# IvanBanny/para-ortho-pca-bo

Hardware: AMD Instinct MI355X
Metric: BO iterations/sec (incl. GP refit + EI opt), BBOB f15 d=40 (higher is better)
Workload: dtype f64; 1 GPU; configs[1]: PCA_BO on BBOB f15 d=40, budget=450, n_DoE=120, EI, var_threshold=0.95; one run per GPU (run list f15/d40/instances 0..N-1 partitioned by pcabo.sharding), timed steps spread evenly over the 330 BO iterations of the run; num_restarts=10, raw_samples=512, batch_limit=5, maxiter=200, parallelism=run-parallel x1

## Files before the change

para-ortho-pca-bo_amd/csrc/kernels_acq.hip:

```cpp
#include "pcabo_internal.h"
#include "acq_math.h"
#include <algorithm>
#include <cstdlib>
#include <mutex>

#define PSTRIDE PCABO_PSTRIDE

#ifdef PCABO_ACQ_TIMING
__device__ unsigned long long g_acq_stamps[16];
#define STAMP(i) do { if (blockIdx.x == gridDim.x / 2 && blockIdx.y == 0 && threadIdx.x == 0) g_acq_stamps[i] = wall_clock64(); } while (0)
#define STAMP_FIN(i) do { if (blockIdx.y == 0 && threadIdx.x == 0) g_acq_stamps[i] = wall_clock64(); } while (0)
extern "C" int pcabo_debug_acq_stamps(unsigned long long* out16) {
  return hipMemcpyFromSymbol(out16, HIP_SYMBOL(g_acq_stamps), sizeof(g_acq_stamps)) == hipSuccess ? 0 : -3;
}
#else
#define STAMP(i)
#define STAMP_FIN(i)
#endif

__device__ inline void st_wt(double* p, double v) {
  __hip_atomic_store(p, v, __ATOMIC_RELAXED, __HIP_MEMORY_SCOPE_AGENT);
}

template <int SLAB>
__device__ inline int slab_row(int s, int m, int NP) {
  return m < SLAB / 2 ? (SLAB / 2) * s + m : NP - (SLAB / 2) * (s + 1) + (m - SLAB / 2);
}

__device__ void acq_finish_query(const double* base, int S, int k, int q, const double* bounds4, const double* ystats,
                                 const AcqParams& p, double* val, double* grad, double* host_val, double* host_grad,
                                 int lane);

__device__ inline void grad_partial_sum(const double* base, int S, int c, int first, double* gs_out, double* gm_out) {
  double gs = 0.0, gm = 0.0;
  int sl = first;
  for (; sl + 21 < S; sl += 24) {
    double a[8], b[8];
#pragma unroll
    for (int t = 0; t < 8; ++t) {
      a[t] = base[(size_t)(sl + 3 * t) * PSTRIDE + 2 + c];
      b[t] = base[(size_t)(sl + 3 * t) * PSTRIDE + 2 + PCABO_MAXD + c];
    }
#pragma unroll
    for (int t = 0; t < 8; ++t) { gs += a[t]; gm += b[t]; }
  }
  {
    double a[8], b[8];
#pragma unroll
    for (int t = 0; t < 8; ++t) {
      const int si = sl + 3 * t;
      const int sc = si < S ? si : 0;
      a[t] = base[(size_t)sc * PSTRIDE + 2 + c];
      b[t] = base[(size_t)sc * PSTRIDE + 2 + PCABO_MAXD + c];
    }
#pragma unroll
    for (int t = 0; t < 8; ++t) { if (sl + 3 * t < S) { gs += a[t]; gm += b[t]; } }
  }
  *gs_out = gs;
  *gm_out = gm;
}

__device__ void acq_finish_scalar(const double* base, int S, int q, const double* ystats, const AcqParams& p, double* val,
                                  double* host_val, double* coef, int lane);
__device__ void acq_scalar_core(double vv, double mus, int q, double ym, double ysd, const AcqParams& p, double* val,
                                double* host_val, double* coef, int l);
template <int SLAB>
__device__ inline void acq_tail(int combine, double* s_v, double* partial, unsigned int* counters, int q, int S, int k,
                                const double* bounds4, const double* ystats, const AcqParams& prm, double* val,
                                double* grad, double* host_val, double* host_grad, HostMirror* hm,
                                unsigned long long seq, int tid, int w, int l) {
  if (!combine) return;
  int* s_flag = reinterpret_cast<int*>(s_v + SLAB);
  STAMP(6);
  asm volatile("s_waitcnt vmcnt(0)" ::: "memory");
  __syncthreads();
  STAMP(7);
  if (tid == 0) {
    unsigned int t = __hip_atomic_fetch_add(&counters[q], 1u, __ATOMIC_RELAXED, __HIP_MEMORY_SCOPE_AGENT);
    int last = ((t % (unsigned int)S) == (unsigned int)(S - 1));
    if (last) {
      __builtin_amdgcn_fence(__ATOMIC_ACQUIRE, "agent");
      asm volatile("s_waitcnt vmcnt(0)" ::: "memory");
    }
    *s_flag = last;
  }
  __syncthreads();
  if (!*s_flag) return;
  STAMP_FIN(8);
  const double* base = partial + (size_t)q * S * PSTRIDE;
  double* s_fin = s_v + SLAB + 2;
  double* s_coef = s_fin + 6 * PCABO_MAXD;
  double rng_c = 1.0;
  if (w == 0) {
    if (prm.want_grad && l < k) rng_c = bounds4[PCABO_MAXD + l] - bounds4[l];
    acq_finish_scalar(base, S, q, ystats, prm, val, host_val, s_coef, l);
  } else if (prm.want_grad) {
    for (int c = l; c < k; c += 64) {
      double gs, gm;
      grad_partial_sum(base, S, c, w - 1, &gs, &gm);
      s_fin[(w - 1) * 2 * PCABO_MAXD + c] = gs;
      s_fin[(w - 1) * 2 * PCABO_MAXD + PCABO_MAXD + c] = gm;
    }
  }
  __syncthreads();
  STAMP_FIN(13);
  if (w == 0) {
    if (prm.want_grad) {
      const double c_mu = s_coef[0], c_sg = s_coef[1];
      for (int c = l; c < k; c += 64) {
        const double gs = (s_fin[c] + s_fin[2 * PCABO_MAXD + c]) + s_fin[4 * PCABO_MAXD + c];
        const double gm = (s_fin[PCABO_MAXD + c] + s_fin[3 * PCABO_MAXD + c]) + s_fin[5 * PCABO_MAXD + c];
        const double g = __fma_rn(c_mu, gm, c_sg * gs) / (c == l ? rng_c : bounds4[PCABO_MAXD + c] - bounds4[c]);
        grad[(size_t)q * k + c] = g;
        if (host_grad) host_grad[(size_t)q * k + c] = g;
      }
    }
    if (hm && l == 0)
      __hip_atomic_store(const_cast<unsigned long long*>(&hm->qflag[q]), seq, __ATOMIC_RELEASE, __HIP_MEMORY_SCOPE_SYSTEM);
    STAMP_FIN(9);
#ifdef PCABO_ACQ_TIMING
    asm volatile("s_waitcnt vmcnt(0)" ::: "memory");
    STAMP_FIN(10);
#endif
  }
}

#define ACQ_BATCH_PROLOGUE()                                                                                     \
  unsigned run_ = blockIdx.z;                                                                                    \
  int qsel_ = -1;                                                                                                \
  if (ab.table) {                                                                                                \
    const unsigned e_ = reinterpret_cast<const unsigned*>(qa.x)[blockIdx.y];                                     \
    run_ = e_ >> 16; qsel_ = (int)(e_ & 0xffffu);                                                                \
  }                                                                                                              \
  if (ab.zs) {                                                                                                   \
    ZnT = zrun(ZnT, ab.zs, run_); R = zrun(R, ab.zs, run_); alpha = zrun(alpha, ab.zs, run_);                    \
    bounds4 = zrun(bounds4, ab.zs, run_); ystats = zrun(ystats, ab.zs, run_); partial = zrun(partial, ab.zs, run_); \
    counters = zrun(counters, ab.zs, run_); val = zrun(val, ab.zs, run_); grad = zrun(grad, ab.zs, run_);        \
    Xq = zrun(Xq, ab.xq_host ? ab.hzs : ab.zs, run_);                                                            \
    host_val = zrun(host_val, ab.hzs, run_); host_grad = zrun(host_grad, ab.hzs, run_); hm = zrun(hm, ab.hzs, run_); \
    if (ab.k_dev) k = *zrun(ab.k_dev, ab.zs, run_);                                                              \
    if (ab.bestf) prm.best_f = *zrun(ab.bestf, ab.zs, run_);                                                     \
    if (ab.hyp) prm.inv_ls = zrun(ab.hyp, ab.zs, run_)[PCABO_HYP_INV_LS];                                        \
  }                                                                                                              \
  (void)qsel_;

template <int SLAB>
__global__ __launch_bounds__(256) void k_acq_fused(
    QueryArgs qa, const double* __restrict__ Xq, int q_total, int n, int k, int NP, int ld,
    const double* __restrict__ ZnT, const double* __restrict__ R, const double* __restrict__ alpha,
    const double* __restrict__ bounds4, const double* __restrict__ ystats, AcqParams prm, double* partial,
    unsigned int* counters, double* __restrict__ val, double* __restrict__ grad,
    double* host_val, double* host_grad, HostMirror* hm, unsigned long long seq, int combine, int ,
    MailPair* , MailPair* , AcqBatch ab) {
  ACQ_BATCH_PROLOGUE()
  const double inv_ls = prm.inv_ls;
  const int kernel = prm.kernel, want_grad = prm.want_grad;
  extern __shared__ __attribute__((aligned(16))) double s_dyn[];
  double* s_ks = s_dyn;
  double* s_cf = s_dyn + NP;
  double* s_tm = s_dyn + 2 * NP;
  double* s_xn = s_dyn + 3 * NP;
  double* s_v = s_xn + PCABO_MAXD;
  const int tid = threadIdx.x, w = tid >> 6, l = tid & 63;
  const int s = blockIdx.x, q = ab.table ? qsel_ : (int)blockIdx.y, S = gridDim.x;
  double* out = partial + ((size_t)q * S + s) * PSTRIDE;
  STAMP(0);

  if (tid < k) {
    double lo = bounds4[tid], hi = bounds4[PCABO_MAXD + tid];
    double xv = Xq ? Xq[(size_t)q * k + tid] : qa.x[q * k + tid];
    s_xn[tid] = (xv - lo) / (hi - lo);
  }
  __syncthreads();
  STAMP(1);
  for (int j = tid; j < NP; j += 256) {
    double ks = 0.0, cf = 0.0;
    if (j < n) {
      double sq = 0.0;
      for (int c = 0; c < k; ++c) { double dlt = s_xn[c] - ZnT[(size_t)c * ld + j]; sq += dlt * dlt; }
      sq *= inv_ls * inv_ls;
      acq_cov(sq, kernel, &ks, &cf);
      cf = cf * inv_ls * inv_ls;
    }
    s_ks[j] = ks;
    s_cf[j] = cf;
  }
  __syncthreads();
  STAMP(2);
  {
    constexpr int RW = SLAB / 4;
    int ri[RW];
    const double* Rr[RW];
    double acc[RW];
    int imax = 0;
#pragma unroll
    for (int u = 0; u < RW; ++u) {
      ri[u] = slab_row<SLAB>(s, w + 4 * u, NP); Rr[u] = R + (size_t)ri[u] * ld; acc[u] = 0.0; imax = max(imax, ri[u]);
    }
    for (int j = l; j <= imax; j += 64) {
      const double kj = s_ks[j];
#pragma unroll
      for (int u = 0; u < RW; ++u) acc[u] += Rr[u][j] * kj;
    }
#pragma unroll
    for (int u = 0; u < RW; ++u) acc[u] = wave_sum(acc[u]);
    if (l == 0) {
#pragma unroll
      for (int u = 0; u < RW; ++u) s_v[w + 4 * u] = acc[u];
    }
  }
  __syncthreads();
  STAMP(3);
  if (w == 0) {
    double vv = 0.0, mu = 0.0;
    if (l < SLAB) {
      const int i = slab_row<SLAB>(s, l, NP);
      const double vi = s_v[l];
      vv = vi * vi;
      if (i < n) mu = alpha[i] * s_ks[i];
    }
    vv = wave_sum(vv);
    mu = wave_sum(mu);
    if (l == 0) { st_wt(out + 0, vv); st_wt(out + 1, mu); }
  }
  if (want_grad) {
  __syncthreads();
  STAMP(4);
  for (int j = tid; j < NP; j += 256) {
    double wj = 0.0;
#pragma unroll
    for (int m = 0; m < SLAB; ++m) wj += R[(size_t)slab_row<SLAB>(s, m, NP) * ld + j] * s_v[m];
    const bool mine = ((j / (SLAB / 2)) == s) || (((NP - 1 - j) / (SLAB / 2)) == s);
    const double cf = s_cf[j];
    s_tm[j] = (mine && j < n) ? alpha[j] * cf : 0.0;
    s_ks[j] = wj * cf;
  }
  __syncthreads();
  STAMP(5);
  for (int c0 = 0; c0 < k; c0 += 32) {
    double gs[8], gm[8], xc[8];
    const double* zrow[8];
#pragma unroll
    for (int u = 0; u < 8; ++u) {
      const int c = c0 + w + 4 * u;
      const int cc = c < k ? c : 0;
      gs[u] = 0.0; gm[u] = 0.0; xc[u] = s_xn[cc]; zrow[u] = ZnT + (size_t)cc * ld;
    }
    for (int j = l; j < n; j += 64) {
      const double ts = s_ks[j], tm = s_tm[j];
#pragma unroll
      for (int u = 0; u < 8; ++u) {
        const double dlt = xc[u] - zrow[u][j];
        gs[u] += ts * dlt;
        gm[u] += tm * dlt;
      }
    }
#pragma unroll
    for (int u = 0; u < 8; ++u) { gs[u] = wave_sum(gs[u]); gm[u] = wave_sum(gm[u]); }
    if (l == 0) {
#pragma unroll
      for (int u = 0; u < 8; ++u) {
        const int c = c0 + w + 4 * u;
        if (c < k) { st_wt(out + 2 + c, gs[u]); st_wt(out + 2 + PCABO_MAXD + c, gm[u]); }
      }
    }
  }
  }

  acq_tail<SLAB>(combine, s_v, partial, counters, q, S, k, bounds4, ystats, prm, val, grad, host_val, host_grad, hm, seq, tid, w, l);
}

#define FIN_STAGE_PER_WAVE (11 * 2 * 40)
__device__ inline bool acq_server_finisher(const MailPair* rec, int S, int k, int q, unsigned long long seq,
                                           const double* ystats, const AcqParams& prm, double* val, double* grad,
                                           double* host_val, double* host_grad, HostMirror* hm, double rng_c,
                                           double* s_fin, double* s_coef, double* s_stage, int* s_srv,
                                           unsigned long long t0, int w, int l) {
  if (w == 0) {
    const double ym = ystats[0], ysd = ystats[1];
    const void* ptr[8];
    pcabo_u4 o[8];
    const MailPair* mine = rec + (size_t)(l < S ? l : 0) * PSTRIDE;
#pragma unroll
    for (int t = 0; t < 8; ++t) ptr[t] = mine + (t & 1);
    for (;;) {
      ld_pairs_sys8(ptr, o);
      const bool ok = pair_tag(o[0]) == seq && pair_tag(o[1]) == seq;
      if (__all(ok)) break;
      if (__any(wall_clock64() - t0 > PCABO_SERVER_TIMEOUT_TICKS)) { if (l == 0) *s_srv = 1; break; }
      __builtin_amdgcn_s_sleep(1);
    }
    double vm[2] = {l < S ? pair_value(o[0]) : 0.0, l < S ? pair_value(o[1]) : 0.0};
    wave_sum_multi<2>(vm, l);
    constexpr int lane_vv = wave_multi_lane(2, 0), lane_mus = wave_multi_lane(2, 1);
    const double vv = read_lane(vm[0], lane_vv), mus = read_lane(vm[0], lane_mus);
    acq_scalar_core(vv, mus, q, ym, ysd, prm, val, host_val, s_coef, l);
  } else if (prm.want_grad) {
    const int first = w - 1;
    const int ns = first < S ? (S - first + 2) / 3 : 0;
    const int total = ns * 2 * k;
    double* stage = s_stage + (size_t)(w - 1) * FIN_STAGE_PER_WAVE;
    for (int i0 = 0; i0 < total; i0 += 512) {
      const void* ptr[8];
      int item[8];
#pragma unroll
      for (int t = 0; t < 8; ++t) {
        const int i = i0 + l + 64 * t;
        item[t] = i < total ? i : -1;
        const int ii = i < total ? i : 0;
        const int st = ii / (2 * k), rem = ii - st * 2 * k, which = rem >= k, c = rem - which * k;
        ptr[t] = rec + (size_t)(first + 3 * st) * PSTRIDE + 2 + which * PCABO_MAXD + c;
      }
      pcabo_u4 o[8];
      for (;;) {
        ld_pairs_sys8(ptr, o);
        bool ok = true;
#pragma unroll
        for (int t = 0; t < 8; ++t) ok = ok && (item[t] < 0 || pair_tag(o[t]) == seq);
        if (__all(ok)) break;
        if (__any(wall_clock64() - t0 > PCABO_SERVER_TIMEOUT_TICKS)) { if (l == 0) *s_srv = 1; break; }
        __builtin_amdgcn_s_sleep(1);
      }
#pragma unroll
      for (int t = 0; t < 8; ++t) if (item[t] >= 0) stage[item[t]] = pair_value(o[t]);
    }
    __builtin_amdgcn_fence(__ATOMIC_RELEASE, "wavefront");
    __builtin_amdgcn_wave_barrier();
    __builtin_amdgcn_fence(__ATOMIC_ACQUIRE, "wavefront");
    if (l < k) {
      double gs = 0.0, gm = 0.0;
      for (int st = 0; st < ns; ++st) { gs += stage[st * 2 * k + l]; gm += stage[st * 2 * k + k + l]; }
      s_fin[(w - 1) * 2 * PCABO_MAXD + l] = gs;
      s_fin[(w - 1) * 2 * PCABO_MAXD + PCABO_MAXD + l] = gm;
    }
  }
  __syncthreads();
  if (*s_srv) return false;
  if (w == 0) {
    if (prm.want_grad && l < k) {
      const double c_mu = s_coef[0], c_sg = s_coef[1];
      const double gs = (s_fin[l] + s_fin[2 * PCABO_MAXD + l]) + s_fin[4 * PCABO_MAXD + l];
      const double gm = (s_fin[PCABO_MAXD + l] + s_fin[3 * PCABO_MAXD + l]) + s_fin[5 * PCABO_MAXD + l];
      const double g = __fma_rn(c_mu, gm, c_sg * gs) / rng_c;
      grad[(size_t)q * k + l] = g;
      if (host_grad) host_grad[(size_t)q * k + l] = g;
    }
    if (hm && l == 0)
      __hip_atomic_store(const_cast<unsigned long long*>(&hm->qflag[q]), seq, __ATOMIC_RELEASE, __HIP_MEMORY_SCOPE_SYSTEM);
  }
  return true;
}

#define FIN_LDS_DOUBLES (6 * PCABO_MAXD + 2 + 3 * FIN_STAGE_PER_WAVE + 2)
__device__ __noinline__ void acq_server_finish_main(double* s_mem, MailPair* dev_mail,
                                                    int ctrl_idx, const MailPair* part_pairs, int S, int k, int q,
                                                    const double* __restrict__ bounds4, const double* __restrict__ ystats,
                                                    const AcqParams& prm, double* val, double* grad, double* host_val,
                                                    double* host_grad, HostMirror* hm, unsigned long long seq) {
  double* s_fin = s_mem;
  int* s_srvp = reinterpret_cast<int*>(s_mem + FIN_LDS_DOUBLES - 1);
  const int tid = threadIdx.x, l = tid & 63;
  const int w = __builtin_amdgcn_readfirstlane(tid >> 6);
  double rng_c = 1.0;
  if (tid < k) rng_c = bounds4[PCABO_MAXD + tid] - bounds4[tid];
  for (unsigned long long cur_seq = seq;; ++cur_seq) {
    const unsigned long long t0 = wall_clock64();
    if (tid == 0) { s_srvp[0] = 0; s_srvp[1] = 0; }
    __syncthreads();
    if (w == 0) {
      for (;;) {
        const pcabo_u4 hd = ld_pair_sys(dev_mail + ctrl_idx);
        if (__all(mail_seq(hd) == cur_seq)) { if (pair_value(hd) == 0.0 && l == 0) *s_srvp = 1; break; }
        if (__any(wall_clock64() - t0 > PCABO_SERVER_TIMEOUT_TICKS)) { if (l == 0) *s_srvp = 1; break; }
        __builtin_amdgcn_s_sleep(1);
      }
    }
    __syncthreads();
    if (*s_srvp) return;
    if (!acq_server_finisher(part_pairs + (size_t)q * S * PSTRIDE, S, k, q, cur_seq, ystats, prm, val, grad, host_val,
                             host_grad, hm, rng_c, s_fin, s_fin + 6 * PCABO_MAXD, s_fin + 6 * PCABO_MAXD + 2, s_srvp, t0, w, l))
      return;
    __syncthreads();
  }
}

#define ACQ_SLAB32_NP 448
int acq_slabs(int NP) { return NP / (NP >= ACQ_SLAB32_NP ? 32 : 16); }

template <int NU, int CU>
__device__ inline void publish_grad(const double (&gs)[CU], const double (&gm)[CU], int w, int k, int l, MailPair* pout,
                                    double* out, unsigned long long seq) {
  static_assert(NU <= CU, "components per wave");
  double v[2 * NU];
#pragma unroll
  for (int u = 0; u < NU; ++u) { v[2 * u] = gs[u]; v[2 * u + 1] = gm[u]; }
  wave_sum_multi<2 * NU>(v, l);
  const int i = wave_multi_owner<2 * NU>(l);
  const int c = w + 4 * (i >> 1);
  if (i >= 0 && c < k) {
    const int off = 2 + (i & 1) * PCABO_MAXD + c;
    if (pout) st_pair_sys(pout + off, make_pair(v[0], seq));
    else st_wt(out + off, v[0]);
  }
}

template <int SLAB, int NB, bool SRV>
__global__ __launch_bounds__(256) void k_acq_fast(
    QueryArgs qa, const double* __restrict__ Xq, int q_total, int n, int k, int NP_rt, int ld,
    const double* __restrict__ ZnT, const double* __restrict__ R, const double* __restrict__ alpha,
    const double* __restrict__ bounds4, const double* __restrict__ ystats, AcqParams prm, double* partial,
    unsigned int* counters, double* __restrict__ val, double* __restrict__ grad,
    double* host_val, double* host_grad, HostMirror* hm, unsigned long long seq, int combine, int qb,
    MailPair* dev_mail, MailPair* part_pairs, AcqBatch ab) {
  if (!SRV) { ACQ_BATCH_PROLOGUE() }
  constexpr int NP = NB * 64;
  constexpr int CU = 10;
  constexpr int RW = SLAB / 4;
  constexpr int NM = (NB + 3) / 4;
  const double inv_ls = prm.inv_ls;
  const int kernel = prm.kernel, want_grad = prm.want_grad;
  extern __shared__ __attribute__((aligned(16))) double s_dyn[];
  double* s_ks = s_dyn;
  double* s_cf = s_dyn + NP;
  double* s_tm = s_dyn + 2 * NP;
  double* s_xn = s_dyn + 3 * NP;
  double* s_v = s_xn + PCABO_MAXD;
  double* s_p4 = s_v + SLAB + 2;
  const int tid = threadIdx.x, l = tid & 63;
  const int w = __builtin_amdgcn_readfirstlane(tid >> 6);
  constexpr bool server = SRV;
  const int s = blockIdx.x, S = server ? (int)gridDim.x - 1 : (int)gridDim.x;
  if (server && s == S) {
    acq_server_finish_main(s_dyn, dev_mail, 1 + q_total * k + (int)blockIdx.y, part_pairs, S, k,
                           blockIdx.y, bounds4, ystats, prm, val, grad, host_val, host_grad, hm, seq);
    return;
  }
  STAMP(0);

  double z[CU][NB], r[RW][NB], al[NM];
  const unsigned lane8 = (unsigned)l * 8u;
#pragma unroll
  for (int u = 0; u < CU; ++u) {
    const int c = w + 4 * u;
    const char* zr = reinterpret_cast<const char*>(ZnT + (size_t)c * ld);
#pragma unroll
    for (int b = 0; b < NB; ++b) {
      z[u][b] = 0.0;
      if (c < k) z[u][b] = *reinterpret_cast<const double*>(zr + lane8 + 512 * b);
    }
  }
#pragma unroll
  for (int u = 0; u < RW; ++u) {
    const int ri = slab_row<SLAB>(s, w + 4 * u, NP);
    const char* Rr = reinterpret_cast<const char*>(R + (size_t)ri * ld);
#pragma unroll
    for (int b = 0; b < NB; ++b) {
      r[u][b] = 0.0;
      if (64 * b <= ri) r[u][b] = *reinterpret_cast<const double*>(Rr + lane8 + 512 * b);
    }
  }
#pragma unroll
  for (int m = 0; m < NM; ++m) { const int j = tid + 256 * m; al[m] = j < n ? alpha[j] : 0.0; }
  int* s_srv = reinterpret_cast<int*>(s_v + SLAB + 1);
  unsigned long long cur_seq = seq;
  double b_lo = 0.0, b_hi = 1.0;
  if (server && l < k) { b_lo = bounds4[l]; b_hi = bounds4[PCABO_MAXD + l]; }
  for (;;) {
  int q = (!SRV && ab.table) ? (int)(reinterpret_cast<const unsigned*>(qa.x)[blockIdx.y] & 0xffffu) : (int)blockIdx.y * qb;
  double* out = partial + ((size_t)q * S + s) * PSTRIDE;
  if (server) {
    const unsigned long long t0 = wall_clock64();
    if (tid == 0) { s_srv[0] = 0; s_srv[1] = 0; }
    __syncthreads();
    if (w == 0) {
      volatile int* flags = s_srv;
      const void* ptr[8];
#pragma unroll
      for (int t = 0; t < 8; ++t) ptr[t] = (t & 1) && l < k ? (const void*)(dev_mail + 1 + q * k + l) : (const void*)(dev_mail + 1 + q_total * k + q);
      for (;;) {
        pcabo_u4 o[8];
        ld_pairs_sys8(ptr, o);
        const bool ctl = mail_seq(o[0]) == cur_seq;
        const bool bye = ctl && pair_value(o[0]) == 0.0;
        const bool ok = ctl && (bye || l >= k || mail_seq(o[1]) == cur_seq);
        if (__all(ok)) {
          if (pair_value(o[0]) == 0.0) { if (l == 0) flags[0] = 1; }
          else if (l < k) s_xn[l] = (pair_value(o[1]) - b_lo) / (b_hi - b_lo);
          break;
        }
        if (__any(wall_clock64() - t0 > PCABO_SERVER_TIMEOUT_TICKS)) { if (l == 0) flags[0] = 1; break; }
        __builtin_amdgcn_s_sleep(1);
      }
    }
    __syncthreads();
    if (*s_srv) return;
  }
  MailPair* pout = server ? part_pairs + ((size_t)q * S + s) * PSTRIDE : nullptr;
  for (int qi = 0; qi < qb; ++qi, ++q, out += (size_t)S * PSTRIDE) {
  if (q >= q_total) break;
  if (qi > 0) __syncthreads();
  if (!server) {
  if (tid < k) {
    double lo = bounds4[tid], hi = bounds4[PCABO_MAXD + tid];
    double xv = Xq ? Xq[(size_t)q * k + tid] : qa.x[q * k + tid];
    s_xn[tid] = (xv - lo) / (hi - lo);
  }
  __syncthreads();
  }
  STAMP(1);
  double xc[CU];
#pragma unroll
  for (int u = 0; u < CU; ++u) xc[u] = s_xn[(w + 4 * u < k) ? w + 4 * u : k - 1];
  {
    double sq[NB];
#pragma unroll
    for (int b = 0; b < NB; ++b) sq[b] = 0.0;
#pragma unroll
    for (int u = 0; u < CU; ++u) {
      if (w + 4 * u < k) {
#pragma unroll
        for (int b = 0; b < NB; ++b) { const double d = xc[u] - z[u][b]; sq[b] += d * d; }
      }
    }
#pragma unroll
    for (int b = 0; b < NB; ++b) s_p4[w * NP + l + 64 * b] = sq[b];
  }
  __syncthreads();
#pragma unroll
  for (int m = 0; m < NM; ++m) {
    const int j = tid + 256 * m;
    if (j < NP) {
      double ks = 0.0, cf = 0.0;
      if (j < n) {
        double sq = ((s_p4[j] + s_p4[NP + j]) + s_p4[2 * NP + j]) + s_p4[3 * NP + j];
        sq *= inv_ls * inv_ls;
        acq_cov(sq, kernel, &ks, &cf);
        cf = cf * inv_ls * inv_ls;
      }
      s_ks[j] = ks;
      s_cf[j] = cf;
    }
  }
  __syncthreads();
  STAMP(2);
  {
    double acc[RW];
#pragma unroll
    for (int u = 0; u < RW; ++u) acc[u] = 0.0;
#pragma unroll
    for (int b = 0; b < NB; ++b) {
      const double kj = s_ks[l + 64 * b];
#pragma unroll
      for (int u = 0; u < RW; ++u) acc[u] += r[u][b] * kj;
    }
    wave_sum_multi<RW>(acc, l);
    const int u = wave_multi_owner<RW>(l);
    if (u >= 0) s_v[w + 4 * u] = acc[0];
  }
  __syncthreads();
  STAMP(3);
  if (w == 0) {
    double vv = 0.0, mu = 0.0;
    if (l < SLAB) {
      const int i = slab_row<SLAB>(s, l, NP);
      const double vi = s_v[l];
      vv = vi * vi;
      if (i < n) mu = alpha[i] * s_ks[i];
    }
    double vm[2] = {vv, mu};
    wave_sum_multi<2>(vm, l);
    const int i = wave_multi_owner<2>(l);
    if (i >= 0) {
      if (server) st_pair_sys(pout + i, make_pair(vm[0], cur_seq));
      else st_wt(out + i, vm[0]);
    }
  }
  if (want_grad) {
  {
    double vw[RW];
#pragma unroll
    for (int u = 0; u < RW; ++u) vw[u] = s_v[w + 4 * u];
#pragma unroll
    for (int b = 0; b < NB; ++b) {
      double pw = 0.0;
#pragma unroll
      for (int u = 0; u < RW; ++u) pw += r[u][b] * vw[u];
      s_p4[w * NP + l + 64 * b] = pw;
    }
  }
  __syncthreads();
  STAMP(4);
#pragma unroll
  for (int m = 0; m < NM; ++m) {
    const int j = tid + 256 * m;
    if (j < NP) {
      const double wj = ((s_p4[j] + s_p4[NP + j]) + s_p4[2 * NP + j]) + s_p4[3 * NP + j];
      const bool mine = ((j / (SLAB / 2)) == s) || (((NP - 1 - j) / (SLAB / 2)) == s);
      const double cf = s_cf[j];
      s_tm[j] = mine ? al[m] * cf : 0.0;
      s_ks[j] = wj * cf;
    }
  }
  __syncthreads();
  STAMP(5);
  {
    double gs[CU], gm[CU];
#pragma unroll
    for (int u = 0; u < CU; ++u) { gs[u] = 0.0; gm[u] = 0.0; }
#pragma unroll
    for (int b = 0; b < NB; ++b) {
      const double ts = s_ks[l + 64 * b], tm = s_tm[l + 64 * b];
#pragma unroll
      for (int u = 0; u < CU; ++u) {
        const double dlt = xc[u] - z[u][b];
        gs[u] += ts * dlt;
        gm[u] += tm * dlt;
      }
    }
    const int nu = k > w ? (k - w + 3) / 4 : 0;
    if (nu > 5) publish_grad<10>(gs, gm, w, k, l, pout, out, cur_seq);
    else if (nu > 2) publish_grad<5>(gs, gm, w, k, l, pout, out, cur_seq);
    else if (nu > 0) publish_grad<2>(gs, gm, w, k, l, pout, out, cur_seq);
  }
  }
  }
  q = (!SRV && ab.table) ? (int)(reinterpret_cast<const unsigned*>(qa.x)[blockIdx.y] & 0xffffu) : (int)blockIdx.y * qb;
  out = partial + ((size_t)q * S + s) * PSTRIDE;
  if (!server) {
    acq_tail<SLAB>(combine, s_v, partial, counters, q, S, k, bounds4, ystats, prm, val, grad, host_val, host_grad, hm, cur_seq, tid, w, l);
    break;
  }
  ++cur_seq;
  __syncthreads();
  }
}

__device__ void acq_scalar_core(double vv, double mus, int q, double ym, double ysd, const AcqParams& p, double* val,
                                double* host_val, double* coef, int l) {
  double value, c_mu, c_sg;
  acq_scalar_chain(vv, mus, ym, ysd, p.best_f, p.maximize, p.acq, &value, &c_mu, &c_sg);
  if (l == 0) {
    val[q] = value;
    if (host_val) host_val[q] = value;
    coef[0] = c_mu;
    coef[1] = c_sg;
  }
  STAMP_FIN(12);
}

__device__ void acq_finish_scalar(const double* base, int S, int q, const double* ystats, const AcqParams& p, double* val,
                                  double* host_val, double* coef, int l) {
  const double ym = ystats[0], ysd = ystats[1];
  double vv = 0.0, mus = 0.0;
  for (int s = l; s < S; s += 64) { vv += base[(size_t)s * PSTRIDE]; mus += base[(size_t)s * PSTRIDE + 1]; }
  vv = wave_sum(vv);
  mus = wave_sum(mus);
  STAMP_FIN(11);
  acq_scalar_core(vv, mus, q, ym, ysd, p, val, host_val, coef, l);
}

__device__ void acq_finish_query(const double* base, int S, int k, int q, const double* bounds4, const double* ystats,
                                 const AcqParams& p, double* val, double* grad, double* host_val, double* host_grad,
                                 int l) {
  __shared__ double s_cf2[4][2];
  double* coef = s_cf2[(threadIdx.x >> 6) & 3];
  acq_finish_scalar(base, S, q, ystats, p, val, host_val, coef, l);
  if (p.want_grad) {
    __builtin_amdgcn_wave_barrier();
    const double c_mu = coef[0], c_sg = coef[1];
    for (int c = l; c < k; c += 64) {
      double a0, b0, a1, b1, a2, b2;
      grad_partial_sum(base, S, c, 0, &a0, &b0);
      grad_partial_sum(base, S, c, 1, &a1, &b1);
      grad_partial_sum(base, S, c, 2, &a2, &b2);
      const double gs = (a0 + a1) + a2, gm = (b0 + b1) + b2;
      double g = __fma_rn(c_mu, gm, c_sg * gs) / (bounds4[PCABO_MAXD + c] - bounds4[c]);
      grad[(size_t)q * k + c] = g;
      if (host_grad) host_grad[(size_t)q * k + c] = g;
    }
  }
}

__global__ __launch_bounds__(256) void k_acq_combine(const double* __restrict__ partial, int q_total, int S, int k,
                                                     const double* __restrict__ bounds4,
                                                     const double* __restrict__ ystats, AcqParams p,
                                                     double* __restrict__ val, double* __restrict__ grad, AcqBatch ab) {
  if (ab.zs) {
    const unsigned run_ = blockIdx.z;
    partial = zrun(partial, ab.zs, run_); bounds4 = zrun(bounds4, ab.zs, run_); ystats = zrun(ystats, ab.zs, run_);
    val = zrun(val, ab.zs, run_); grad = zrun(grad, ab.zs, run_);
    if (ab.k_dev) k = *zrun(ab.k_dev, ab.zs, run_);
    if (ab.bestf) p.best_f = *zrun(ab.bestf, ab.zs, run_);
  }
  const int q = blockIdx.x * 4 + (threadIdx.x >> 6);
  if (q < q_total)
    acq_finish_query(partial + (size_t)q * S * PSTRIDE, S, k, q, bounds4, ystats, p, val, grad, nullptr, nullptr,
                     threadIdx.x & 63);
}

#ifdef PCABO_ACQ_TIMING
#define GSTAMP(i) do { if (blockIdx.x == gridDim.x - 1 && blockIdx.y == 0 && threadIdx.x == 0) g_acq_stamps[i] = wall_clock64(); } while (0)
#else
#define GSTAMP(i)
#endif
#define GQ 5
#define GT_LD 17
#define WAVE_LDS_SYNC() asm volatile("s_waitcnt lgkmcnt(0)" ::: "memory")
template <int NT>
__global__ __launch_bounds__(256) void k_acq_group(
    QueryArgs qa, const double* __restrict__ Xq, int n, int k, int NP, int ld,
    const double* __restrict__ ZnT, const double* __restrict__ R, const double* __restrict__ alpha,
    const double* __restrict__ bounds4, const double* __restrict__ ystats, AcqParams prm, double* partial,
    unsigned int* counters, double* __restrict__ val, double* __restrict__ grad, double* host_val, double* host_grad,
    HostMirror* hm, unsigned long long seq, AcqBatch ab) {
  const unsigned ent = reinterpret_cast<const unsigned*>(qa.x)[blockIdx.y];
  const unsigned run_ = ent >> 16;
  const int q0 = (int)((ent >> 8) & 0xffu), nq = (int)(ent & 0xffu);
  if (ab.zs) {
    ZnT = zrun(ZnT, ab.zs, run_); R = zrun(R, ab.zs, run_); alpha = zrun(alpha, ab.zs, run_);
    bounds4 = zrun(bounds4, ab.zs, run_); ystats = zrun(ystats, ab.zs, run_); partial = zrun(partial, ab.zs, run_);
    counters = zrun(counters, ab.zs, run_); val = zrun(val, ab.zs, run_); grad = zrun(grad, ab.zs, run_);
    Xq = zrun(Xq, ab.xq_host ? ab.hzs : ab.zs, run_);
    host_val = zrun(host_val, ab.hzs, run_); host_grad = zrun(host_grad, ab.hzs, run_); hm = zrun(hm, ab.hzs, run_);
    if (ab.k_dev) k = *zrun(ab.k_dev, ab.zs, run_);
    if (ab.bestf) prm.best_f = *zrun(ab.bestf, ab.zs, run_);
    if (ab.hyp) prm.inv_ls = zrun(ab.hyp, ab.zs, run_)[PCABO_HYP_INV_LS];
  }
  const int tid = threadIdx.x, l = tid & 63;
  const int w = __builtin_amdgcn_readfirstlane(tid >> 6);
  const int s = blockIdx.x, S = gridDim.x;
  const int r0 = 64 * s, ncol = 64 * (s + 1);
  const int KS = (k + 1) & ~1;
  extern __shared__ __attribute__((aligned(16))) double s_dyn[];
  double* s_ks = s_dyn;
  double* s_tile = s_ks + GQ * (NP > 2 * KS ? NP : 2 * KS);
  double* s_v = s_tile + 4 * 64 * GT_LD;
  double* s_tm = s_v + 64 * 8;
  double* s_coef = s_tm + GQ * 64;
  int* s_flag = reinterpret_cast<int*>(s_coef + 2 * GQ);
  double* s_vvmu = s_coef + 2 * GQ + 4;
  double* s_xn = s_vvmu + 2 * GQ;
  double* s_part = s_tile;
  double* s_gout = s_ks;
  const double inv_ls = prm.inv_ls;
  const int kernel = prm.kernel;

  GSTAMP(0);
  for (int idx = tid; idx < GQ * k; idx += 256) {
    const int q = idx / k, c = idx - q * k;
    const int qq = q < nq ? q : 0;
    const double lo = bounds4[c], hi = bounds4[PCABO_MAXD + c];
    s_xn[q * KS + c] = (Xq[(size_t)(q0 + qq) * k + c] - lo) / (hi - lo);
  }
  __syncthreads();
  GSTAMP(1);
  double cfr[NT][GQ];
  {
    const int jlim = n < ncol ? n : ncol;
    double sq[NT][GQ];
#pragma unroll
    for (int t = 0; t < NT; ++t)
#pragma unroll
      for (int q = 0; q < GQ; ++q) sq[t][q] = 0.0;
    constexpr int CB = NT == 1 ? 40 : (NT == 2 ? 20 : 8);
    for (int c0 = 0; c0 < k; c0 += CB) {
      double z[NT][CB];
#pragma unroll
      for (int t = 0; t < NT; ++t)
#pragma unroll
        for (int u = 0; u < CB; ++u) {
          const int cc = c0 + u < k ? c0 + u : k - 1, jj = tid + 256 * t < NP ? tid + 256 * t : NP - 1;
          z[t][u] = ZnT[(size_t)cc * ld + jj];
        }
#pragma unroll
      for (int u = 0; u < CB; ++u) {
        if (c0 + u < k) {
#pragma unroll
          for (int q = 0; q < GQ; ++q) {
            const double xq = s_xn[q * KS + c0 + u];
#pragma unroll
            for (int t = 0; t < NT; ++t) { const double d = xq - z[t][u]; sq[t][q] += d * d; }
          }
        }
      }
    }
#pragma unroll
    for (int t = 0; t < NT; ++t) {
      const int j = tid + 256 * t;
#pragma unroll
      for (int q = 0; q < GQ; ++q) {
        double ks = 0.0, cf = 0.0;
        if (j < jlim) {
          acq_cov(sq[t][q] * (inv_ls * inv_ls), kernel, &ks, &cf);
          cf = cf * inv_ls * inv_ls;
        }
        if (j < NP) s_ks[q * NP + j] = ks;
        cfr[t][q] = cf;
      }
    }
  }
  __syncthreads();
  GSTAMP(2);
  {
    double acc[GQ];
#pragma unroll
    for (int q = 0; q < GQ; ++q) acc[q] = 0.0;
    const int nblk = s + 1;
    const double* Rs = R + (size_t)r0 * ld + 16 * w + (l & 15);
    double* tw = s_tile + w * 64 * GT_LD;
    auto fetch = [&](int J, double (&dst)[16]) {
#pragma unroll
      for (int u = 0; u < 16; ++u) dst[u] = Rs[(size_t)(4 * u + (l >> 4)) * ld + 64 * J];
    };
    auto put = [&](const double (&src)[16]) {
#pragma unroll
      for (int u = 0; u < 16; ++u) tw[(4 * u + (l >> 4)) * GT_LD + (l & 15)] = src[u];
      WAVE_LDS_SYNC();
    };
    auto use = [&](int J) {
      const double* trow = tw + l * GT_LD;
      const double* kcol = s_ks + 64 * J + 16 * w;
#pragma unroll
      for (int jj = 0; jj < 16; ++jj) {
        const double rv = trow[jj];
#pragma unroll
        for (int q = 0; q < GQ; ++q) acc[q] += rv * kcol[q * NP + jj];
      }
      WAVE_LDS_SYNC();
    };
    double bufA[16], bufB[16];
    fetch(0, bufA);
    if (nblk > 1) fetch(1, bufB);
    for (int J = 0; J < nblk; J += 2) {
      put(bufA);
      if (J + 2 < nblk) fetch(J + 2, bufA);
      use(J);
      if (J + 1 < nblk) {
        put(bufB);
        if (J + 3 < nblk) fetch(J + 3, bufB);
        use(J + 1);
      }
    }
#pragma unroll
    for (int q = 0; q < GQ; ++q) s_part[w * 64 * GT_LD + q * 64 + l] = acc[q];
  }
  __syncthreads();
  for (int idx = tid; idx < GQ * 64; idx += 256) {
    const int q = idx >> 6, m = idx & 63;
    const double* pp = s_part + q * 64 + m;
    s_v[m * 8 + q] = ((pp[0] + pp[64 * GT_LD]) + pp[2 * 64 * GT_LD]) + pp[3 * 64 * GT_LD];
  }
  __syncthreads();
  GSTAMP(3);
  for (int q = w; q < nq; q += 4) {
    const int i = r0 + l;
    const double vi = s_v[l * 8 + q];
    double vv = vi * vi;
    double mu = i < n ? alpha[i] * s_ks[q * NP + i] : 0.0;
    vv = wave_sum(vv);
    mu = wave_sum(mu);
    if (l == 0) { s_vvmu[2 * q] = vv; s_vvmu[2 * q + 1] = mu; }
  }
  if (prm.want_grad) {
    double wacc[NT][GQ];
#pragma unroll
    for (int t = 0; t < NT; ++t)
#pragma unroll
      for (int q = 0; q < GQ; ++q) wacc[t][q] = 0.0;
    constexpr int RU = NT <= 2 ? 16 : 8;
    for (int m0 = 0; m0 < 64; m0 += RU) {
      double rr[RU][NT];
#pragma unroll
      for (int u = 0; u < RU; ++u)
#pragma unroll
        for (int t = 0; t < NT; ++t) {
          const int j = tid + 256 * t;
          const double rv = R[(size_t)(r0 + m0 + u) * ld + (j < ncol ? j : 0)];
          rr[u][t] = j < ncol ? rv : 0.0;
        }
#pragma unroll
      for (int u = 0; u < RU; ++u) {
        double vq[GQ];
#pragma unroll
        for (int q = 0; q < GQ; ++q) vq[q] = s_v[(m0 + u) * 8 + q];
#pragma unroll
        for (int t = 0; t < NT; ++t)
#pragma unroll
          for (int q = 0; q < GQ; ++q) wacc[t][q] += rr[u][t] * vq[q];
      }
    }
    GSTAMP(4);
    __syncthreads();
#pragma unroll
    for (int t = 0; t < NT; ++t) {
      const int j = tid + 256 * t;
      if (j < NP) {
        const bool mine = j >= r0 && j < r0 + 64;
        const double aj = (mine && j < n) ? alpha[j] : 0.0;
#pragma unroll
        for (int q = 0; q < GQ; ++q) {
          s_ks[q * NP + j] = wacc[t][q] * cfr[t][q];
          if (mine) s_tm[q * 64 + (j - r0)] = aj * cfr[t][q];
        }
      }
    }
    __syncthreads();
    GSTAMP(5);
    constexpr int NBL = 4 * NT;
    const int jmax = n < ncol ? n : ncol;
    double ts[GQ][NBL], tmq[GQ];
#pragma unroll
    for (int b = 0; b < NBL; ++b) {
      const int j = l + 64 * b;
#pragma unroll
      for (int q = 0; q < GQ; ++q) ts[q][b] = j < jmax ? s_ks[q * NP + j] : 0.0;
    }
#pragma unroll
    for (int q = 0; q < GQ; ++q) tmq[q] = (r0 + l < n) ? s_tm[q * 64 + l] : 0.0;
    __syncthreads();
    GSTAMP(10);
    double zc[NBL], zn_[NBL];
    auto load_row = [&](int c, double (&dst)[NBL]) {
      const double* zrow = ZnT + (size_t)c * ld;
#pragma unroll
      for (int b = 0; b < NBL; ++b) dst[b] = zrow[(64 * b < jmax) ? l + 64 * b : l];
    };
    if (w < k) load_row(w, zc);
    for (int c = w; c < k; c += 4) {
      if (c + 4 < k) load_row(c + 4, zn_);
      if (c == w) { GSTAMP(11); }
      double gs[GQ], gm[GQ];
      const int bm = r0 >> 6;
#pragma unroll
      for (int q = 0; q < GQ; ++q) {
        const double xq = s_xn[q * KS + c];
        double a = 0.0, zm = 0.0;
// ... 430 lines not shown
```

Measured before the change: 402.0 BO iterations/s.

## Split persistent acquisition server rounds into specialized loop templated on component count

The persistent server path of the acquisition kernel moves into a separate function, acq_resident_rounds. It is templated on the number of active components per wave, so the inner loops run only the needed component count instead of a runtime-guarded CU=10. Row indices and alpha values are hoisted out of the loop, explicit FMAs are used, and xc is optionally reloaded to ease register pressure. Server stamp instrumentation is added under the timing macro. The non-server path loses its server branches, which may shrink code and register usage, at the cost of more template instantiations and slightly different rounding.

```diff
diff --git a/para-ortho-pca-bo_amd/csrc/kernels_acq.hip b/para-ortho-pca-bo_amd/csrc/kernels_acq.hip
--- a/para-ortho-pca-bo_amd/csrc/kernels_acq.hip
+++ b/para-ortho-pca-bo_amd/csrc/kernels_acq.hip
@@ -13,9 +13,18 @@
 extern "C" int pcabo_debug_acq_stamps(unsigned long long* out16) {
   return hipMemcpyFromSymbol(out16, HIP_SYMBOL(g_acq_stamps), sizeof(g_acq_stamps)) == hipSuccess ? 0 : -3;
 }
+__device__ unsigned long long g_srv_stamps[256][16];
+#define SRV_STAMP(i, sq) do { if (blockIdx.y == 0 && threadIdx.x == 0 && blockIdx.x == ((i) < 8 ? (gridDim.x - 1) / 2 : gridDim.x - 1)) { \
+    g_srv_stamps[(sq) & 255][i] = wall_clock64(); if ((i) == 0) g_srv_stamps[(sq) & 255][15] = (sq); } } while (0)
+extern "C" int pcabo_debug_srv_stamps(unsigned long long* out4096) {
+  if (hipMemcpyFromSymbol(out4096, HIP_SYMBOL(g_srv_stamps), sizeof(g_srv_stamps)) != hipSuccess) return -3;
+  void* d = nullptr;
+  return hipGetSymbolAddress(&d, HIP_SYMBOL(g_srv_stamps)) == hipSuccess && hipMemset(d, 0, sizeof(g_srv_stamps)) == hipSuccess ? 0 : -3;
+}
 #else
 #define STAMP(i)
 #define STAMP_FIN(i)
+#define SRV_STAMP(i, sq)
 #endif
 
 __device__ inline void st_wt(double* p, double v) {
@@ -290,11 +299,13 @@
       if (__any(wall_clock64() - t0 > PCABO_SERVER_TIMEOUT_TICKS)) { if (l == 0) *s_srv = 1; break; }
       __builtin_amdgcn_s_sleep(1);
     }
+    SRV_STAMP(9, seq);
     double vm[2] = {l < S ? pair_value(o[0]) : 0.0, l < S ? pair_value(o[1]) : 0.0};
     wave_sum_multi<2>(vm, l);
     constexpr int lane_vv = wave_multi_lane(2, 0), lane_mus = wave_multi_lane(2, 1);
     const double vv = read_lane(vm[0], lane_vv), mus = read_lane(vm[0], lane_mus);
     acq_scalar_core(vv, mus, q, ym, ysd, prm, val, host_val, s_coef, l);
+    SRV_STAMP(10, seq);
   } else if (prm.want_grad) {
     const int first = w - 1;
     const int ns = first < S ? (S - first + 2) / 3 : 0;
@@ -336,6 +347,7 @@
   }
   __syncthreads();
   if (*s_srv) return false;
+  SRV_STAMP(11, seq);
   if (w == 0) {
     if (prm.want_grad && l < k) {
       const double c_mu = s_coef[0], c_sg = s_coef[1];
@@ -347,6 +359,10 @@
     }
     if (hm && l == 0)
       __hip_atomic_store(const_cast<unsigned long long*>(&hm->qflag[q]), seq, __ATOMIC_RELEASE, __HIP_MEMORY_SCOPE_SYSTEM);
+#ifdef PCABO_ACQ_TIMING
+    asm volatile("s_waitcnt vmcnt(0)" ::: "memory");
+    SRV_STAMP(12, seq);
+#endif
   }
   return true;
 }
@@ -377,6 +393,7 @@
     }
     __syncthreads();
     if (*s_srvp) return;
+    SRV_STAMP(8, cur_seq);
     if (!acq_server_finisher(part_pairs + (size_t)q * S * PSTRIDE, S, k, q, cur_seq, ystats, prm, val, grad, host_val,
                              host_grad, hm, rng_c, s_fin, s_fin + 6 * PCABO_MAXD, s_fin + 6 * PCABO_MAXD + 2, s_srvp, t0, w, l))
       return;
@@ -401,6 +418,201 @@
     const int off = 2 + (i & 1) * PCABO_MAXD + c;
     if (pout) st_pair_sys(pout + off, make_pair(v[0], seq));
     else st_wt(out + off, v[0]);
+  }
+}
+
+template <int NUC, int NB>
+__device__ __forceinline__ void round_sqdist(const double (&z)[10][NB], const double (&xc)[10], double (&sq)[NB]) {
+#pragma clang fp contract(off)
+#pragma unroll
+  for (int b = 0; b < NB; ++b) {
+    sq[b] = 0.0;
+    if (NUC > 0) { const double d = xc[0] - z[0][b]; sq[b] = d * d; }
+  }
+#pragma unroll
+  for (int u = 1; u < NUC; ++u) {
+#pragma unroll
+    for (int b = 0; b < NB; ++b) { const double d = xc[u] - z[u][b]; sq[b] = __builtin_fma(d, d, sq[b]); }
+  }
+}
+template <int RW, int NB>
+__device__ __forceinline__ void round_rows_dot(const double (&r)[RW][NB], const double* s_ks, int l, double (&acc)[RW]) {
+#pragma clang fp contract(off)
+#pragma unroll
+  for (int u = 0; u < RW; ++u) acc[u] = 0.0;
+#pragma unroll
+  for (int b = 0; b < NB; ++b) {
+    const double kj = s_ks[l + 64 * b];
+#pragma unroll
+    for (int u = 0; u < RW; ++u) acc[u] = __builtin_fma(r[u][b], kj, acc[u]);
+  }
+}
+template <int RW, int NB>
+__device__ __forceinline__ void round_cols_dot(const double (&r)[RW][NB], const double (&vw)[RW], double* s_out, int l) {
+#pragma clang fp contract(off)
+#pragma unroll
+  for (int b = 0; b < NB; ++b) {
+    double pw = 0.0;
+#pragma unroll
+    for (int u = 0; u < RW; ++u) pw = __builtin_fma(r[u][b], vw[u], pw);
+    s_out[l + 64 * b] = pw;
+  }
+}
+template <int NUC, int NB>
+__device__ __forceinline__ void round_contract(const double (&z)[10][NB], const double (&xc)[10], const double* s_ts,
+                                               const double* s_tm, int l, double* gs, double* gm) {
+#pragma clang fp contract(off)
+#pragma unroll
+  for (int u = 0; u < NUC; ++u) { gs[u] = 0.0; gm[u] = 0.0; }
+#pragma unroll
+  for (int b = 0; b < NB; ++b) {
+    const double ts = s_ts[l + 64 * b], tm = s_tm[l + 64 * b];
+#pragma unroll
+    for (int u = 0; u < NUC; ++u) {
+      const double dlt = xc[u] - z[u][b];
+      gs[u] = __builtin_fma(ts, dlt, gs[u]);
+      gm[u] = __builtin_fma(tm, dlt, gm[u]);
+    }
+  }
+}
+template <int KIND, int NP, int NM>
+__device__ __forceinline__ void round_cov_columns(const double* s_p4, double* s_ks, double* s_cf, int n, int tid, double inv_ls) {
+#pragma unroll
+  for (int m = 0; m < NM; ++m) {
+    const int j = tid + 256 * m;
+    if (j < NP) {
+      double ks = 0.0, cf = 0.0;
+      if (j < n) {
+        double sq = ((s_p4[j] + s_p4[NP + j]) + s_p4[2 * NP + j]) + s_p4[3 * NP + j];
+        sq *= inv_ls * inv_ls;
+        acq_cov(sq, KIND, &ks, &cf);
+        cf = cf * inv_ls * inv_ls;
+      }
+      s_ks[j] = ks;
+      s_cf[j] = cf;
+    }
+  }
+}
+
+template <int SLAB, int NB, int NUC>
+__device__ __forceinline__ void acq_resident_rounds(const double (&z)[10][NB], const double (&r)[SLAB / 4][NB],
+                                                    const double (&al)[(NB + 3) / 4], double* s_dyn, int s, int S, int q,
+                                                    int q_total, int n, int k, double inv_ls, int kernel,
+                                                    const double* __restrict__ alpha, const double* __restrict__ bounds4,
+                                                    MailPair* dev_mail, MailPair* part_pairs, unsigned long long seq,
+                                                    int tid, int w, int l) {
+  constexpr int NP = NB * 64, CU = 10, RW = SLAB / 4, NM = (NB + 3) / 4;
+  constexpr bool RELOAD_XC = NB >= 5;
+  double* s_ks = s_dyn;
+  double* s_cf = s_dyn + NP;
+  double* s_tm = s_dyn + 2 * NP;
+  double* s_xn = s_dyn + 3 * NP;
+  double* s_v = s_xn + PCABO_MAXD;
+  double* s_p4 = s_v + SLAB + 2;
+  int* s_srv = reinterpret_cast<int*>(s_v + SLAB + 1);
+  double b_lo = 0.0, b_hi = 1.0;
+  if (l < k) { b_lo = bounds4[l]; b_hi = bounds4[PCABO_MAXD + l]; }
+  if (tid >= k && tid < 4 * CU) s_xn[tid] = 0.0;
+  const int row_l = slab_row<SLAB>(s, l < SLAB ? l : 0, NP);
+  double al_row = 0.0;
+  if (w == 0 && l < SLAB && row_l < n) al_row = alpha[row_l];
+  MailPair* pout = part_pairs + ((size_t)q * S + s) * PSTRIDE;
+  const void* ptr[8];
+#pragma unroll
+  for (int t = 0; t < 8; ++t) ptr[t] = (t & 1) && l < k ? (const void*)(dev_mail + 1 + q * k + l) : (const void*)(dev_mail + 1 + q_total * k + q);
+  for (unsigned long long cur_seq = seq;; ++cur_seq) {
+    const unsigned long long t0 = wall_clock64();
+    if (tid == 0) { s_srv[0] = 0; s_srv[1] = 0; }
+    __syncthreads();
+    if (w == 0) {
+      volatile int* flags = s_srv;
+      for (;;) {
+        pcabo_u4 o[8];
+        ld_pairs_sys8(ptr, o);
+        const bool ctl = mail_seq(o[0]) == cur_seq;
+        const bool bye = ctl && pair_value(o[0]) == 0.0;
+        const bool ok = ctl && (bye || l >= k || mail_seq(o[1]) == cur_seq);
+        if (__all(ok)) {
+          if (pair_value(o[0]) == 0.0) { if (l == 0) flags[0] = 1; }
+          else if (l < k) s_xn[l] = (pair_value(o[1]) - b_lo) / (b_hi - b_lo);
+          break;
+        }
+        if (__any(wall_clock64() - t0 > PCABO_SERVER_TIMEOUT_TICKS)) { if (l == 0) flags[0] = 1; break; }
+        __builtin_amdgcn_s_sleep(1);
+      }
+    }
+    __syncthreads();
+    if (*s_srv) return;
+    SRV_STAMP(0, cur_seq);
+    double xc[CU];
+#pragma unroll
+    for (int u = 0; u < CU; ++u) xc[u] = u < NUC ? s_xn[w + 4 * u] : 0.0;
+    {
+      double sq[NB];
+      round_sqdist<NUC, NB>(z, xc, sq);
+#pragma unroll
+      for (int b = 0; b < NB; ++b) s_p4[w * NP + l + 64 * b] = sq[b];
+    }
+    SRV_STAMP(1, cur_seq);
+    __syncthreads();
+    if (kernel == 1) round_cov_columns<1, NP, NM>(s_p4, s_ks, s_cf, n, tid, inv_ls);
+    else round_cov_columns<0, NP, NM>(s_p4, s_ks, s_cf, n, tid, inv_ls);
+    __syncthreads();
+    SRV_STAMP(2, cur_seq);
+    {
+      double acc[RW];
+      round_rows_dot<RW, NB>(r, s_ks, l, acc);
+      wave_sum_multi<RW>(acc, l);
+      const int u = wave_multi_owner<RW>(l);
+      if (u >= 0) s_v[w + 4 * u] = acc[0];
+    }
+    __syncthreads();
+    SRV_STAMP(3, cur_seq);
+    if (w == 0) {
+      double vv = 0.0, mu = 0.0;
+      if (l < SLAB) {
+        const double vi = s_v[l];
+        vv = vi * vi;
+        if (row_l < n) mu = al_row * s_ks[row_l];
+      }
+      double vm[2] = {vv, mu};
+      wave_sum_multi<2>(vm, l);
+      const int i = wave_multi_owner<2>(l);
+      if (i >= 0) st_pair_sys(pout + i, make_pair(vm[0], cur_seq));
+    }
+    SRV_STAMP(4, cur_seq);
+    {
+      double vw[RW];
+#pragma unroll
+      for (int u = 0; u < RW; ++u) vw[u] = s_v[w + 4 * u];
+      round_cols_dot<RW, NB>(r, vw, s_p4 + w * NP, l);
+    }
+    __syncthreads();
+    SRV_STAMP(5, cur_seq);
+#pragma unroll
+    for (int m = 0; m < NM; ++m) {
+      const int j = tid + 256 * m;
+      if (j < NP) {
+        const double wj = ((s_p4[j] + s_p4[NP + j]) + s_p4[2 * NP + j]) + s_p4[3 * NP + j];
+        const bool mine = ((j / (SLAB / 2)) == s) || (((NP - 1 - j) / (SLAB / 2)) == s);
+        const double cf = s_cf[j];
+        s_tm[j] = mine ? al[m] * cf : 0.0;
+        s_ks[j] = wj * cf;
+      }
+    }
+    __syncthreads();
+    SRV_STAMP(6, cur_seq);
+    if constexpr (NUC > 0) {
+      double gs[NUC > 0 ? NUC : 1], gm[NUC > 0 ? NUC : 1];
+      if constexpr (RELOAD_XC) {
+#pragma unroll
+        for (int u = 0; u < CU; ++u) xc[u] = u < NUC ? s_xn[w + 4 * u] : 0.0;
+      }
+      round_contract<NUC, NB>(z, xc, s_ks, s_tm, l, gs, gm);
+      publish_grad<(NUC > 0 ? NUC : 1)>(gs, gm, w, k, l, pout, nullptr, cur_seq);
+    }
+    SRV_STAMP(7, cur_seq);
+    __syncthreads();
   }
 }
 
@@ -461,52 +673,28 @@
   }
 #pragma unroll
   for (int m = 0; m < NM; ++m) { const int j = tid + 256 * m; al[m] = j < n ? alpha[j] : 0.0; }
-  int* s_srv = reinterpret_cast<int*>(s_v + SLAB + 1);
-  unsigned long long cur_seq = seq;
-  double b_lo = 0.0, b_hi = 1.0;
-  if (server && l < k) { b_lo = bounds4[l]; b_hi = bounds4[PCABO_MAXD + l]; }
-  for (;;) {
-  int q = (!SRV && ab.table) ? (int)(reinterpret_cast<const unsigned*>(qa.x)[blockIdx.y] & 0xffffu) : (int)blockIdx.y * qb;
+  if constexpr (SRV) {
+    const int nu = k > w ? (k - w + 3) / 4 : 0;
+#define ACQ_ROUNDS(NUC) acq_resident_rounds<SLAB, NB, NUC>(z, r, al, s_dyn, s, S, (int)blockIdx.y, q_total, n, k, inv_ls, kernel, \
+                                                           alpha, bounds4, dev_mail, part_pairs, seq, tid, w, l)
+    if (nu > 5) ACQ_ROUNDS(10);
+    else if (nu > 2) ACQ_ROUNDS(5);
+    else if (nu > 0) ACQ_ROUNDS(2);
+    else ACQ_ROUNDS(0);
+#undef ACQ_ROUNDS
+    return;
+  } else {
+  int q = ab.table ? (int)(reinterpret_cast<const unsigned*>(qa.x)[blockIdx.y] & 0xffffu) : (int)blockIdx.y * qb;
   double* out = partial + ((size_t)q * S + s) * PSTRIDE;
-  if (server) {
-    const unsigned long long t0 = wall_clock64();
-    if (tid == 0) { s_srv[0] = 0; s_srv[1] = 0; }
-    __syncthreads();
-    if (w == 0) {
-      volatile int* flags = s_srv;
-      const void* ptr[8];
-#pragma unroll
-      for (int t = 0; t < 8; ++t) ptr[t] = (t & 1) && l < k ? (const void*)(dev_mail + 1 + q * k + l) : (const void*)(dev_mail + 1 + q_total * k + q);
-      for (;;) {
-        pcabo_u4 o[8];
-        ld_pairs_sys8(ptr, o);
-        const bool ctl = mail_seq(o[0]) == cur_seq;
-        const bool bye = ctl && pair_value(o[0]) == 0.0;
-        const bool ok = ctl && (bye || l >= k || mail_seq(o[1]) == cur_seq);
-        if (__all(ok)) {
-          if (pair_value(o[0]) == 0.0) { if (l == 0) flags[0] = 1; }
-          else if (l < k) s_xn[l] = (pair_value(o[1]) - b_lo) / (b_hi - b_lo);
-          break;
-        }
-        if (__any(wall_clock64() - t0 > PCABO_SERVER_TIMEOUT_TICKS)) { if (l == 0) flags[0] = 1; break; }
-        __builtin_amdgcn_s_sleep(1);
-      }
-    }
-    __syncthreads();
-    if (*s_srv) return;
-  }
-  MailPair* pout = server ? part_pairs + ((size_t)q * S + s) * PSTRIDE : nullptr;
   for (int qi = 0; qi < qb; ++qi, ++q, out += (size_t)S * PSTRIDE) {
   if (q >= q_total) break;
   if (qi > 0) __syncthreads();
-  if (!server) {
   if (tid < k) {
     double lo = bounds4[tid], hi = bounds4[PCABO_MAXD + tid];
     double xv = Xq ? Xq[(size_t)q * k + tid] : qa.x[q * k + tid];
     s_xn[tid] = (xv - lo) / (hi - lo);
   }
   __syncthreads();
-  }
   STAMP(1);
   double xc[CU];
 #pragma unroll
@@ -570,10 +758,7 @@
     double vm[2] = {vv, mu};
     wave_sum_multi<2>(vm, l);
     const int i = wave_multi_owner<2>(l);
-    if (i >= 0) {
-      if (server) st_pair_sys(pout + i, make_pair(vm[0], cur_seq));
-      else st_wt(out + i, vm[0]);
-    }
+    if (i >= 0) st_wt(out + i, vm[0]);
   }
   if (want_grad) {
   {
@@ -618,20 +803,14 @@
       }
     }
     const int nu = k > w ? (k - w + 3) / 4 : 0;
-    if (nu > 5) publish_grad<10>(gs, gm, w, k, l, pout, out, cur_seq);
-    else if (nu > 2) publish_grad<5>(gs, gm, w, k, l, pout, out, cur_seq);
-    else if (nu > 0) publish_grad<2>(gs, gm, w, k, l, pout, out, cur_seq);
-  }
-  }
-  }
-  q = (!SRV && ab.table) ? (int)(reinterpret_cast<const unsigned*>(qa.x)[blockIdx.y] & 0xffffu) : (int)blockIdx.y * qb;
-  out = partial + ((size_t)q * S + s) * PSTRIDE;
-  if (!server) {
-    acq_tail<SLAB>(combine, s_v, partial, counters, q, S, k, bounds4, ystats, prm, val, grad, host_val, host_grad, hm, cur_seq, tid, w, l);
-    break;
-  }
-  ++cur_seq;
-  __syncthreads();
+    if (nu > 5) publish_grad<10>(gs, gm, w, k, l, nullptr, out, seq);
+    else if (nu > 2) publish_grad<5>(gs, gm, w, k, l, nullptr, out, seq);
+    else if (nu > 0) publish_grad<2>(gs, gm, w, k, l, nullptr, out, seq);
+  }
+  }
+  }
+  q = ab.table ? (int)(reinterpret_cast<const unsigned*>(qa.x)[blockIdx.y] & 0xffffu) : (int)blockIdx.y * qb;
+  acq_tail<SLAB>(combine, s_v, partial, counters, q, S, k, bounds4, ystats, prm, val, grad, host_val, host_grad, hm, seq, tid, w, l);
   }
 }
 
```

Result: no change. 408.3 BO iterations/s (median of 6 runs) (+1.6%).
